# Sanoojan/VFace

Measured on AMD Instinct MI355X. Metric: swapped frames/sec at 512x512, 50-step DDIM, higher is better.
Workload: dtype f16

## Files before the change

### include/vface_hip.h

```cpp
#ifndef VFACE_HIP_H
#define VFACE_HIP_H

#include <stddef.h>
#include <stdint.h>

#ifdef __cplusplus
extern "C" {
#endif

#define VFACE_ABI_VERSION 7

#define VFACE_OK 0
#define VFACE_ERR_ARG (-1)
#define VFACE_ERR_ALIGN (-2)
#define VFACE_ERR_SHAPE (-3)
#define VFACE_ERR_DTYPE (-4)
#define VFACE_ERR_LAUNCH (-5)
#define VFACE_ERR_WORKSPACE (-6)

#define VFACE_F16 0
#define VFACE_BF16 1

#define VFACE_EPI_GEGLU 1
#define VFACE_EPI_OUT_F32 2
#define VFACE_TUNE_VARIANT(v) ((v) << 8)
#define VFACE_CONV_PAD_TRAILING 0x40000
#define VFACE_TUNE_NO_PERSISTENT 0x10000
#define VFACE_TUNE_PERSISTENT 0x20000
#define VFACE_TUNE_NO_PATCH 0x80000
#define VFACE_TUNE_PATCH 0x100000
#define VFACE_TUNE_GN8 0x8000000
#define VFACE_TUNE_NO_Q8 0x4000000
#define VFACE_TUNE_PATCH_BN160 0x2000000
#define VFACE_TUNE_F32_TRANSPOSE 0x1000000
#define VFACE_TUNE_BIG_TILE 0x10000000
#define VFACE_TUNE_NO_BIG_TILE 0x20000000
#define VFACE_TUNE_BIG_W256 0x200000
#define VFACE_TUNE_BIG_W320 0x400000

#define VFACE_FUSION_NONE 0
#define VFACE_FUSION_REPLACE 1
#define VFACE_FUSION_LINEAR 2

int vface_abi_version(void);
const char* vface_error_string(int code);
int vface_gemm_variants_built(void);

typedef struct vface_stream32 {
    const float* residual32;
    int64_t ldr32;
    float* out32;
    int64_t ldo32;
    const float* in_scale_shift;
    int64_t ld_scale_shift;
    int in_silu;
} vface_stream32;

int vface_gemm(const void* A, int64_t lda, const void* A2, int64_t lda2, int K1, int a2_row_mod, const void* Wt,
               int64_t ldw, int M, int N, int K, const float* bias, const float* rowbias, int rows_per_sample,
               int ld_rowbias, const void* residual, int64_t ldr, void* C, int64_t ldc, const void* zeros, int flags,
               int dtype, float* colstats, int64_t ld_colstats, void* workspace, int64_t workspace_bytes, void* stream,
               const vface_stream32* s32);

int64_t vface_splitk_workspace_bytes(int M, int N, int K, int flags, int rows_per_sample);

int vface_conv3x3(const void* X, int64_t ldx, int nimg, int H, int W, int Cin, const void* Wt, int64_t ldw, int Cout,
                  int stride, int upsample, const float* bias, const float* rowbias, int ld_rowbias,
                  const void* residual, int64_t ldr, void* Y, int64_t ldy, const void* zeros, int flags, int dtype,
                  float* colstats, int64_t ld_colstats, void* workspace, int64_t workspace_bytes, void* stream,
                  const vface_stream32* s32);

int vface_conv_uses_patch_kernel(int H, int W, int Cin, int Cout, int window, int stride, int upsample, int flags);

int vface_conv3x3_plus_1x1(const void* X, int64_t ldx, int nimg, int H, int W, int Cin, const void* X2, int64_t ldx2, int C2,
                           const void* Wt, int64_t ldw, int Cout, const float* bias, const float* rowbias, int ld_rowbias,
                           void* Y, int64_t ldy, const void* zeros, int flags, int dtype, float* colstats,
                           int64_t ld_colstats, void* workspace, int64_t workspace_bytes, void* stream,
                           const vface_stream32* s32);

int vface_upsample2x_conv3x3_phase(const void* X, int64_t ldx, int nimg, int H, int W, int Cin, const void* Wt, int64_t ldw,
                                   int Cout, int py, int px, const float* bias, const float* rowbias, int ld_rowbias, void* Y,
                                   int64_t ldy, const void* zeros, int flags, int dtype, float* colstats,
                                   int64_t ld_colstats, void* stream, const vface_stream32* s32);

int vface_attention(const void* Q, const void* K, const void* V, int64_t ldq, int64_t ldk, int64_t ldv, int64_t bsq,
                    int64_t bsk, int64_t bsv, const int32_t* qk_map, const int32_t* v_map, void* O, int64_t ldo,
                    int64_t bso, int B, int heads, int n, int nk, int dh, float scale, int dtype, int v_sets,
                    int set_stride, void* stream);
int vface_attention_shared_scores_supported(int dh, int v_sets);

int vface_layernorm(const void* x, int64_t ldx, const float* gamma, const float* beta, void* y, int64_t ldy, int M,
// ... 131 lines not shown
```

### vface_amd/csrc/gemm.hip

```cpp
#include <type_traits>

#include "common.hpp"
#include "vface_kernels.hpp"

namespace {

constexpr int BM = 128, BK = 64;
enum { MODE_PLAIN = 0, MODE_CONV_FAST = 1, MODE_CONV_GENERIC = 2 };

template <class TT, int MODE, int NT, bool DB, bool PERSIST, int RM = -1>
__global__ __launch_bounds__(256, 2) void gemm_kernel(GemmParams p) {
    using E = typename TT::elem;
    using V8 = typename TT::v8;
    constexpr int BN = 32 * NT;
    constexpr int BROUNDS = BN / 32;
    constexpr int A_ELEMS = BM * BK, B_ELEMS = BN * BK, STAGE = A_ELEMS + B_ELEMS;
    extern __shared__ __attribute__((aligned(16))) unsigned char smem_raw[];
    E* smem = reinterpret_cast<E*>(smem_raw);

    const int t = threadIdx.x;
    const int lane = t & 63;
    const int wave = __builtin_amdgcn_readfirstlane(t >> 6);
    const int wm = wave >> 1, wn = wave & 1;
    unsigned long long dbg_t0 = 0, dbg_t1 = 0, dbg_t2 = 0, dbg_e0 = 0, dbg_ew = 0, dbg_er = 0, dbg_es = 0;
// ... 800 lines not shown

template <class TT>
int launch_gemm(const GemmParams& p, int variant, hipStream_t stream) {
    if (p.mode == 0) return launch_mode<TT, MODE_PLAIN>(p, variant, stream);
    if (p.Cin % 64 == 0) return launch_mode<TT, MODE_CONV_FAST>(p, variant, stream);
    return launch_mode<TT, MODE_CONV_GENERIC>(p, variant, stream);
}

int pick_variant(const GemmParams& p) {
    const int forced = (p.flags >> 8) & 0xF;
    if (forced) return forced;
    const bool geglu = p.flags & GEMM_GEGLU;
    const long mref = p.rows_per_sample > 1 ? 24L * p.rows_per_sample : p.M;
    const long tiles160 = ((mref + BM - 1) / BM) * (p.N / 160);
    const bool n160 = !geglu && (p.N % 160 == 0) && ((p.N % 128 != 0) || tiles160 >= 1536);
    return n160 ? 6 : 5;
}

int split_for(int M, int N, int K, int flags, int rows_per_sample) {
    if (flags & (GEMM_GEGLU | GEMM_OUT_F32)) return 1;
    if ((N & 7) || ((flags >> 8) & 0xF) == 0xF) return 1;
    const bool n160 = (N % 160 == 0) && (N % 128 != 0);
    const int bn = n160 ? 160 : 128;
    const long mref = rows_per_sample > 1 ? 24L * rows_per_sample : M;
    const int tiles = (int)((mref + BM - 1) / BM) * ((N + bn - 1) / bn);
    const int nt = (K + BK - 1) / BK;
    if (tiles > 192 || nt < 16) return 1;
    int s = 512 / tiles;
    if (s > 8) s = 8;
    if (s > nt / 8) s = nt / 8;
    return s < 2 ? 1 : s;
}

}

int vf_launch_gemm_bf16(const GemmParams& p, int variant, hipStream_t stream);
#if defined(VF_GEMM_TU) && VF_GEMM_TU == 1
int vf_launch_gemm_bf16(const GemmParams& p, int variant, hipStream_t stream) { return launch_gemm<BF16>(p, variant, stream); }
#else
bool vf_gemm_variants_built() { return false; }

long vf_splitk_workspace_bytes(int M, int N, int K, int flags, int rows_per_sample) {
    int s = split_for(M, N, K, flags, rows_per_sample);
    if (s < 2) s = 0;
    if (rows_per_sample == 64 && (N % 128) == 0 && !(flags & (GEMM_GEGLU | GEMM_OUT_F32))) {
        int s8 = (int)(256 / (12L * (N / 128)));
        if (s8 > 8) s8 = 8;
        if (s8 < 1) s8 = 1;
        if (s8 > s) s = s8;
    }
    return (long)s * M * N * 4;
}

int vf_launch_gemm(const GemmParams& p_in, int dtype, hipStream_t stream) {
    GemmParams p = p_in;
    p.split_k = 1; p.kt_per_split = 0;
    if (!p.A || !p.Wt || (!p.C && !p.C32) || !p.zeros) return VF_ERR_ARG;
    if (p.M <= 0 || p.N <= 0 || p.K <= 0) return VF_ERR_ARG;
    if (p.res_f32 && !p.residual) p.res_f32 = 0;
    if (p.res_f32 || p.C32) {
        if ((p.flags & (GEMM_GEGLU | GEMM_OUT_F32 | GEMM_NARROW_EPILOGUE | 0x4000)) || (p.N & 7)) return VF_ERR_SHAPE;
        if (p.C32 && (((uintptr_t)p.C32 & 15) || (p.ldc32 & 3))) return VF_ERR_ALIGN;
        if (p.res_f32 && (((uintptr_t)p.residual & 15) || (p.ldr & 3))) return VF_ERR_ALIGN;
        if (p.out_phase && p.res_f32) return VF_ERR_SHAPE;
    }
    if ((p.K & 7) || (p.Kw & 7) || (p.lda & 7) || (p.ldw & 7) || (p.N & 3) || (p.ldc & 3)) return VF_ERR_ALIGN;
    if (((uintptr_t)p.A | (uintptr_t)p.Wt | (uintptr_t)p.zeros) & 15) return VF_ERR_ALIGN;
    if ((uintptr_t)p.C & 7) return VF_ERR_ALIGN;
    if (p.C32 && (((uintptr_t)p.C & 15) || (p.ldc & 7))) return VF_ERR_ALIGN;
    if (p.residual && (((uintptr_t)p.residual & 7) || (p.ldr & 3))) return VF_ERR_ALIGN;
    if (p.rowbias && (p.rows_per_sample <= 0 || (p.ld_rowbias & 3))) return VF_ERR_ARG;
    if ((p.flags & GEMM_GEGLU) && ((p.N & 31) || (p.flags & GEMM_OUT_F32) || p.residual || p.rowbias)) return VF_ERR_SHAPE;
    if (p.colstats && ((p.flags & (GEMM_GEGLU | GEMM_OUT_F32)) || (p.ld_colstats & 1) || ((uintptr_t)p.colstats & 15))) return VF_ERR_ARG;
    if (p.A2 && (p.K1 <= 0 || (p.K1 % BK) || (p.lda2 & 7) || ((uintptr_t)p.A2 & 15))) return VF_ERR_ALIGN;
    if (p.A2 && p.mode == 1 && ((p.Cin % 64) || ((p.K - p.K1) % BK) || p.upsample || p.a2_row_mod)) return VF_ERR_SHAPE;
    if (p.mode == 1) {
        if (p.ntaps == 0) { p.KH = p.KW = 3; p.ntaps = 9; p.pad_x = p.pad; }
        if (p.Cin <= 0 || (p.Cin & 7) || p.ntaps != p.KH * p.KW || p.ntaps > 9) return VF_ERR_SHAPE;
        if (p.A2 ? (p.K1 != p.ntaps * p.Cin || p.K <= p.K1) : (p.K != p.ntaps * p.Cin)) return VF_ERR_SHAPE;
        if (p.out_phase && (p.residual || (p.flags & GEMM_OUT_F32) || (p.N & 7))) return VF_ERR_SHAPE;
        if (p.out_phase && p.colstats && ((p.OH * p.OW) & 63)) return VF_ERR_SHAPE;
        if (p.stride != 1 && p.stride != 2) return VF_ERR_SHAPE;
    }
    {
        const unsigned long es = 2, lim = 0xFFFFFFF0ul;
        const unsigned long rows = p.mode == 1 ? (unsigned long)(p.M / (p.OH * p.OW)) * p.H * p.W : (unsigned long)p.M;
        const unsigned long ab = ((rows - 1) * (unsigned long)p.lda + (p.mode == 1 ? p.Cin : (p.A2 ? p.K1 : p.K))) * es;
        const unsigned long wb = ((unsigned long)(p.N - 1) * p.ldw + p.Kw) * es;
        unsigned long a2b = 0;
        if (p.A2) a2b = ((unsigned long)((p.a2_row_mod > 0 ? p.a2_row_mod : p.M) - 1) * p.lda2 + (p.K - p.K1)) * es;
        if (ab >= lim || wb >= lim || a2b >= lim) return VF_ERR_SHAPE;
        p.a_bytes = (unsigned)ab; p.w_bytes = (unsigned)wb; p.a2_bytes = (unsigned)a2b;
    }
    if (p.gn_ab) {
        if (p.mode != 1 || p.M <= 0) return VF_ERR_SHAPE;
        const unsigned long nimg = (unsigned long)(p.M / (p.OH * p.OW));
        const unsigned long gb = ((nimg - 1) * (unsigned long)p.ld_gn_ab + p.Cin) * 8ul;
        if (gb >= 0xFFFFFFF0ul) return VF_ERR_SHAPE;
        p.gn_ab_bytes = (unsigned)gb;
    }
    if (vf_conv_in16_ok(p)) return vf_launch_conv_in16(p, dtype, stream);
    int karg = 0;
    const int kchoice = vf_conv_kernel_choice(p, &karg);
    if (kchoice == 1) return vf_launch_conv_patch(p, dtype, stream);
    if (kchoice == 2 && p.workspace) {
        const int s = karg;
        if (s && p.workspace_bytes >= (long)s * p.M * p.N * 4 && !((uintptr_t)p.workspace & 15) && (p.M % 64) == 0 &&
            !(p.residual && (((uintptr_t)p.residual & 15) || (p.ldr & 7))) && !(p.ldc & 7) && !((uintptr_t)p.C & 15)) {
            p.split_k = s;
            const int rc = vf_launch_conv_q8(p, dtype, stream);
            if (rc != VF_OK) return rc;
            if (dtype == VF_DTYPE_F16) hipLaunchKernelGGL(splitk_reduce_kernel<F16>, dim3((p.M + 63) / 64, (p.N + 255) / 256), dim3(256), 0, stream, p);
            else hipLaunchKernelGGL(splitk_reduce_kernel<BF16>, dim3((p.M + 63) / 64, (p.N + 255) / 256), dim3(256), 0, stream, p);
            return hipGetLastError() == hipSuccess ? VF_OK : VF_ERR_LAUNCH;
        }
    }
    if (p.mode == 0 && (p.flags & GEMM_PATCH) && !((p.flags >> 8) & 0xF) && vf_gemm_patch_tile(p)) return vf_launch_gemm_patch(p, dtype, stream);
    if (p.mode == 0 && vf_gemm_big_choice(p)) return vf_launch_gemm_big(p, dtype, stream);
    if (p.gn_ab) return VF_ERR_SHAPE;
    const int variant = pick_variant(p);
    if ((p.res_f32 || p.C32) && variant != 5 && variant != 6) return VF_ERR_SHAPE;
    if (p.mode == 1 && (p.ntaps != 9 || p.out_phase || p.A2) && variant != 5 && variant != 6) return VF_ERR_SHAPE;
    if (p.workspace && !p.out_phase && (variant == 5 || variant == 6) && !((p.flags >> 8) & 0xF) && !(p.flags & 0x4000)) {
        const int s = split_for(p.M, p.N, p.K, p.flags, p.rows_per_sample);
        if (s > 1 && p.workspace_bytes >= (long)s * p.M * p.N * 4 && !((uintptr_t)p.workspace & 15) &&
            !(p.residual && (((uintptr_t)p.residual & 15) || (p.ldr & 7))) && !(p.ldc & 7) && !((uintptr_t)p.C & 15)) {
            const int nt = (p.K + BK - 1) / BK;
            p.split_k = s;
            p.kt_per_split = (nt + s - 1) / s;
            if ((long)(s - 1) * p.kt_per_split >= nt) p.split_k = (nt + p.kt_per_split - 1) / p.kt_per_split;
        }
    }
    if ((p.flags & GEMM_GEGLU) && (variant == 2 || variant == 4 || variant == 6 || variant == 8 || variant == 10)) return VF_ERR_SHAPE;
    if (p.colstats && (variant < 5 || variant > 8)) return VF_ERR_SHAPE;
    if ((variant >= 1 && variant <= 4) || variant == 9 || variant == 10) return VF_ERR_SHAPE;
    if (dtype == VF_DTYPE_F16) return launch_gemm<F16>(p, variant, stream);
    if (dtype == VF_DTYPE_BF16) return vf_launch_gemm_bf16(p, variant, stream);
    return VF_ERR_DTYPE;
}
#endif
```

### vface_amd/csrc/gemm_big.hip

```cpp
#include <type_traits>

#include "common.hpp"
#include "vface_kernels.hpp"

namespace {

constexpr int BM2 = 256, BN2 = 320;
constexpr int A_BYTES = BM2 * 128, B_BYTES = BN2 * 128, STAGE_BYTES = A_BYTES + B_BYTES;

template <class TT, int EPI, int NJ = 10>
__global__ __launch_bounds__(512, 2) void gemm256_kernel(GemmParams p) {
    static_assert(NJ == 10 || (NJ == 8 && EPI != 3), "channel tiles per wave");
    constexpr int BN2 = 32 * NJ, WN = 16 * NJ;
    constexpr int B_BYTES = BN2 * 128, STAGE_BYTES = A_BYTES + B_BYTES;
    constexpr int NPC = 4 + NJ / 2, NS = 2 * NJ;
    using E = typename TT::elem;
    using V8 = typename TT::v8;
    using V4 = typename TT::v4;
    extern __shared__ __attribute__((aligned(16))) unsigned char smem_raw[];
    const int t = threadIdx.x;
    const int lane = t & 63;
    const int wave = __builtin_amdgcn_readfirstlane(t >> 6);
    const int wm = wave >> 1, wn = wave & 1;
    const int fr = lane & 15, fq = lane >> 4;
    constexpr unsigned OOB = 0xFFFFFFF0u;

    const int ntn = p.N / BN2, ntm = (p.M + BM2 - 1) / BM2;
    int m0, n0;
    {
        const int nwg = ntn * ntm, id = blockIdx.x;
        const int q = nwg >> 3, r = nwg & 7, xcd = id & 7, loc = id >> 3;
        const int L = (xcd < r ? xcd * (q + 1) : r * (q + 1) + (xcd - r) * q) + loc;
        const int GN = p.tile_group > 0 ? p.tile_group : 8;
        const int g = L / (GN * ntm);
        const int rem = L - g * (GN * ntm);
        const int gw = min(GN, ntn - g * GN);
        const int tm = rem / gw;
        m0 = tm * BM2;
        n0 = (g * GN + (rem - tm * gw)) * BN2;
    }

    const float* rowbias_row = nullptr;
    if constexpr (EPI == 3) {
        const int rps = max(p.rows_per_sample, 1);
        const int smp = __builtin_amdgcn_readfirstlane(m0 / rps);
        rowbias_row = p.rowbias ? p.rowbias + (long)smp * p.ld_rowbias : nullptr;
    }
    const i32x4_t rA = raw_buffer_rsrc(p.A, p.a_bytes);
    const i32x4_t rA2 = raw_buffer_rsrc(p.A2 ? p.A2 : p.A, p.A2 ? p.a2_bytes : 0u);
    const i32x4_t rW = raw_buffer_rsrc(p.Wt, p.w_bytes);

    unsigned a_off[4], a2_off[4], b_off[NJ / 2];
#pragma unroll
    for (int i = 0; i < 4; ++i) {
        const int row = (wave + 8 * i) * 8 + (lane >> 3);
        const unsigned ch = (unsigned)((lane & 7) ^ ((row >> 1) & 7));
        const long m = m0 + row;
        a_off[i] = m < p.M ? (unsigned)((m * p.lda + ch * 8) * 2) : OOB;
        a2_off[i] = (p.A2 && m < p.M) ? (unsigned)((m * p.lda2 + ch * 8) * 2) : OOB;
    }
#pragma unroll
    for (int i = 0; i < NJ / 2; ++i) {
        const int row = (wave + 8 * i) * 8 + (lane >> 3);
        const unsigned ch = (unsigned)((lane & 7) ^ ((row >> 1) & 7));
        b_off[i] = (unsigned)((((long)(n0 + row)) * p.ldw + ch * 8) * 2);
    }
    const unsigned lds0 = lds_addr_of(smem_raw);
    auto issue_piece = [&](int s, int kt, int buf) {
        const unsigned kbase = (unsigned)kt * 64u;
        if (s < 4) {
            const bool second = p.A2 && (int)kbase >= p.K1;
            const unsigned base = second ? a2_off[s] : a_off[s];
            const unsigned off = base != OOB ? base + (second ? kbase - (unsigned)p.K1 : kbase) * 2u : OOB;
            const unsigned dst = lds0 + (unsigned)buf * STAGE_BYTES + (unsigned)(wave + 8 * s) * 1024u;
            if (second) raw_lds_dma16(rA2, dst, (int)off, 0);
            else raw_lds_dma16(rA, dst, (int)off, 0);
        } else {
            const unsigned dst = lds0 + (unsigned)buf * STAGE_BYTES + A_BYTES + (unsigned)(wave + 8 * (s - 4)) * 1024u;
            raw_lds_dma16(rW, dst, (int)(b_off[s - 4] + kbase * 2u), 0);
        }
    };

    f4_t acc[NJ][4];
#pragma unroll
    for (int j = 0; j < NJ; ++j)
#pragma unroll
        for (int i = 0; i < 4; ++i) acc[j][i] = f4_t{0.f, 0.f, 0.f, 0.f};

    const int arow = wm * 64 + fr, wrow = wn * WN + fr;
    const unsigned aadr = (unsigned)(arow * 128 + ((fq ^ ((arow >> 1) & 7)) << 4));
    const unsigned wadr = (unsigned)(A_BYTES + wrow * 128 + ((fq ^ ((wrow >> 1) & 7)) << 4));

    const int nt = p.K >> 6;
#pragma unroll
    for (int s = 0; s < NPC; ++s) issue_piece(s, 0, 0);
    if (nt > 1) { issue_piece(0, 1, 1); issue_piece(1, 1, 1); }
// ... 24 lines not shown
                if (s2 < NS) {
                    const int kk2 = s2 / NJ, j2 = s2 - kk2 * NJ;
                    wf[s2 & 3] = *reinterpret_cast<const V8*>(st + ((wadr + j2 * 2048) ^ (kk2 ? 64u : 0u)));
                } else if (more) {
                    wf[s2 & 3] = *reinterpret_cast<const V8*>(sn + wadr + (s2 - NS) * 2048);
                }
            }
            if (s == 4) {
#pragma unroll
                for (int i = 0; i < 4; ++i) af[1][i] = *reinterpret_cast<const V8*>(st + ((aadr + i * 2048) ^ 64u));
            }
            if (s == NS - 2 && more) {
#pragma unroll
                for (int i = 0; i < 4; ++i) af[0][i] = *reinterpret_cast<const V8*>(sn + aadr + i * 2048);
            }
            if (s >= NS - 2) { if (more2) issue_piece(s - (NS - 2), kt + 2, cur); }
            else if (s < NPC - 2) { if (more) issue_piece(s + 2, kt + 1, cur ^ 1); }
            __builtin_amdgcn_sched_barrier(0);
            __builtin_amdgcn_s_setprio(1);
#pragma unroll
            for (int i = 0; i < 4; ++i) acc[j][i] = TT::mfma32(wf[s & 3], af[kk][i], acc[j][i]);
            __builtin_amdgcn_s_setprio(0);
            __builtin_amdgcn_sched_barrier(0);
        }
    }

    __syncthreads();
    {
    int te = threadIdx.x;
    asm volatile("" : "+v"(te));
    const int lane = te & 63, fr = lane & 15, fq = lane >> 4;
    const int wrow0 = m0 + wm * 64;
    {
        auto add_vec = [&](const float* vec) {
            const __amdgpu_buffer_rsrc_t rV = __builtin_amdgcn_make_buffer_rsrc(const_cast<void*>(vec ? (const void*)vec : p.Wt), 0, vec ? p.N * 4 : 0, 0x00020000);
#pragma unroll
            for (int jh = 0; jh < 2; ++jh) {
                constexpr int HJ = NJ / 2;
                f4_t bj[HJ];
#pragma unroll
                for (int j = 0; j < HJ; ++j)
                    bj[j] = __builtin_bit_cast(f4_t, __builtin_amdgcn_raw_buffer_load_b128(rV, (n0 + wn * WN + (jh * HJ + j) * 16 + fq * 4) * 4, 0, 0));
#pragma unroll
                for (int j = 0; j < HJ; ++j)
#pragma unroll
                    for (int i = 0; i < 4; ++i) {
                        acc[jh * HJ + j][i] += bj[j];
                        asm volatile("" : "+v"(acc[jh * HJ + j][i]));
                    }
                __builtin_amdgcn_sched_barrier(0);
            }
        };
        add_vec(p.bias);
        if constexpr (EPI == 3) {
            add_vec(rowbias_row);
        }
    }
    __builtin_amdgcn_sched_barrier(0);
    E* Cout = reinterpret_cast<E*>(p.C);
    if constexpr (EPI == 0 || EPI == 1) {
        constexpr int OW = EPI == 1 ? WN / 2 : WN;
        constexpr int CH = OW / 8;
        constexpr int SPH = OW * 2 + 16;
        constexpr int NIT = (16 * CH + 63) / 64;
        unsigned char* scr = smem_raw + wave * (16 * SPH);
        const int ncol0 = EPI == 1 ? ((n0 + wn * WN) >> 1) : (n0 + wn * WN);
        int rr[NIT], cc[NIT];
#pragma unroll
        for (int it = 0; it < NIT; ++it) {
            const int idx = lane + 64 * it;
            rr[it] = idx < 16 * CH ? idx / CH : -1;
            cc[it] = idx - (idx / CH) * CH;
        }
#pragma unroll
        for (int i = 0; i < 4; ++i) {
            unsigned char* hrow = scr + fr * SPH + fq * 8;
            if constexpr (EPI == 0) {
#pragma unroll
                for (int j = 0; j < NJ; ++j)
                    *reinterpret_cast<V4*>(hrow + j * 32) = V4{from_f32<E>(acc[j][i][0]), from_f32<E>(acc[j][i][1]), from_f32<E>(acc[j][i][2]), from_f32<E>(acc[j][i][3])};
            } else {
#pragma unroll
                for (int jj = 0; jj < NJ / 2; ++jj) {
                    const float a0 = acc[2 * jj][i][0], a1 = acc[2 * jj][i][1], a2 = acc[2 * jj][i][2], a3 = acc[2 * jj][i][3];
                    const float g0 = acc[2 * jj + 1][i][0], g1 = acc[2 * jj + 1][i][1], g2 = acc[2 * jj + 1][i][2], g3 = acc[2 * jj + 1][i][3];
                    *reinterpret_cast<V4*>(hrow + jj * 32) = V4{from_f32<E>(a0 * gelu_erf_f(g0)), from_f32<E>(a1 * gelu_erf_f(g1)),
                                                                from_f32<E>(a2 * gelu_erf_f(g2)), from_f32<E>(a3 * gelu_erf_f(g3))};
                }
            }
            V8 o[NIT];
#pragma unroll
            for (int it = 0; it < NIT; ++it) o[it] = *reinterpret_cast<const V8*>(scr + max(rr[it], 0) * SPH + cc[it] * 16);
#pragma unroll
            for (int it = 0; it < NIT; ++it) {
                const long m = wrow0 + i * 16 + rr[it];
                if (rr[it] >= 0 && m < p.M) *reinterpret_cast<V8*>(Cout + m * p.ldc + ncol0 + cc[it] * 8) = o[it];
            }
        }
    } else if constexpr (EPI == 3) {
        constexpr int SP = 84;
        float* scr = reinterpret_cast<float*>(smem_raw) + wave * (16 * SP);
        const __amdgpu_buffer_rsrc_t rR = __builtin_amdgcn_make_buffer_rsrc(const_cast<void*>(p.residual ? p.residual : p.Wt), 0, (int)(p.residual ? p.res_bytes : 0u), 0x00020000);
        const __amdgpu_buffer_rsrc_t rC = __builtin_amdgcn_make_buffer_rsrc(p.C ? p.C : const_cast<void*>(p.Wt), 0, (int)(p.C ? p.c_bytes : 0u), 0x00020000);
        const __amdgpu_buffer_rsrc_t rC32 = __builtin_amdgcn_make_buffer_rsrc(p.C32, 0, (int)p.c32_bytes, 0x00020000);
        const int rrow = lane / 10, rch = lane - rrow * 10;
        const bool act = lane < 60;
        const bool has_res = p.residual != nullptr, has_c16 = p.C != nullptr;
// ... 104 lines not shown
                r32[it][1] = __builtin_bit_cast(f4_t, __builtin_amdgcn_raw_buffer_load_b128(rR, (int)off, 16, 0));
            }
        };
#pragma unroll
        for (int i = 0; i < 4; ++i) {
            float* srow = scr + fr * SP + fq * 4;
#pragma unroll
            for (int j = 0; j < NJ; ++j)
                *reinterpret_cast<float4*>(srow + j * 16) = make_float4(acc[j][i][0], acc[j][i][1], acc[j][i][2], acc[j][i][3]);
            __builtin_amdgcn_sched_barrier(0);
            if (i == 0) {
#pragma unroll
                for (int it = 0; it < NPASS; ++it) load_res(0, it);
            }
#pragma unroll
            for (int it = 0; it < NPASS; ++it) {
                const unsigned char* lrd = reinterpret_cast<const unsigned char*>(scr) + lofs[it];
                const f4_t x0 = *reinterpret_cast<const f4_t*>(lrd), x1 = *reinterpret_cast<const f4_t*>(lrd + 16);
                const f4_t a = r32[it][0], b = r32[it][1];
                const long m = wrow0 + i * 16 + rr[it];
                V8 o;
                o[0] = from_f32<E>(x0[0] + a[0]); o[1] = from_f32<E>(x0[1] + a[1]); o[2] = from_f32<E>(x0[2] + a[2]); o[3] = from_f32<E>(x0[3] + a[3]);
                o[4] = from_f32<E>(x1[0] + b[0]); o[5] = from_f32<E>(x1[1] + b[1]); o[6] = from_f32<E>(x1[2] + b[2]); o[7] = from_f32<E>(x1[3] + b[3]);
                if (i + 1 < 4) load_res(i + 1, it);
                const unsigned off = m < p.M ? (unsigned)((m * p.ldc + ncol0 + cc[it] * 8) * 2) : OOB;
                __builtin_amdgcn_raw_buffer_store_b128(__builtin_bit_cast(i32x4_t, o), rC, (int)off, 0, 0);
                __builtin_amdgcn_sched_barrier(0);
            }
        }
    }
    }
}

template <class TT, int EPI, int NJ>
int launch_big(const GemmParams& p, hipStream_t stream) {
    auto kern = gemm256_kernel<TT, EPI, NJ>;
    static VfOncePerDevice attr_set;
    constexpr int BN = 32 * NJ;
    constexpr int lds = 2 * (A_BYTES + BN * 128);
    if (!attr_set.set_lds(reinterpret_cast<const void*>(kern), lds)) return VF_ERR_LAUNCH;
    const int ntn = p.N / BN, ntm = (p.M + BM2 - 1) / BM2;
    GemmParams q = p;
    {
        const double a_mt = (double)BM2 * p.K * 2.0, w_nt = (double)BN * p.K * 2.0;
        int gn = (int)(__builtin_sqrt((double)ntm * ntn / 8.0 * a_mt / w_nt) + 0.5);
        const int cap = (int)(2097152.0 / w_nt);
        if (gn > cap) gn = cap;
        q.tile_group = gn < 1 ? 1 : (gn > ntn ? ntn : gn);
    }
    hipLaunchKernelGGL(kern, dim3(ntn * ntm), dim3(512), lds, stream, q);
    return hipGetLastError() == hipSuccess ? VF_OK : VF_ERR_LAUNCH;
}

template <class TT, int EPI>
int launch_big_width(const GemmParams& p, hipStream_t stream) {
    if constexpr (EPI != 3) {
        bool w256 = false;
        if (p.N % 256 == 0 && !(p.flags & GEMM_BIG_W320)) {
            const long ntm = (p.M + BM2 - 1) / BM2;
            const long r320 = (ntm * (p.N / 320) + 255) / 256, r256 = (ntm * (p.N / 256) + 255) / 256;
            w256 = (p.flags & GEMM_BIG_W256) || (p.K <= 1280 && (double)r256 * 0.85 < (double)r320);
        }
        if (w256) return launch_big<TT, EPI, 8>(p, stream);
    }
    return launch_big<TT, EPI, 10>(p, stream);
}

template <class TT>
int launch_big_dtype(const GemmParams& p, hipStream_t stream) {
    if (p.C32) return launch_big_width<TT, 3>(p, stream);
    if (p.flags & GEMM_GEGLU) return launch_big_width<TT, 1>(p, stream);
    if (p.residual) return launch_big_width<TT, 2>(p, stream);
    return launch_big_width<TT, 0>(p, stream);
}

}

bool vf_gemm_big_ok(const GemmParams& p) {
    if (p.mode != 0 || p.out_phase || p.gn_ab || p.split_k > 1 || p.a2_row_mod) return false;
    if ((p.N % BN2) || (p.K & 63) || p.K < 128 || (p.Kw < p.K)) return false;
    if (p.A2 && ((p.K1 & 63) || p.K1 <= 0 || p.K1 >= p.K)) return false;
    if (p.flags & (GEMM_OUT_F32 | GEMM_NARROW_EPILOGUE | GEMM_F32_TRANSPOSE | 0x4000 | (0xF << 8))) return false;
    if (p.C32) {
        if (p.flags & GEMM_GEGLU) return false;
        if (((uintptr_t)p.C32 & 15) || (p.ldc32 & 3)) return false;
        if (p.rowbias && (p.rows_per_sample <= 0 || (p.rows_per_sample % BM2) || (p.ld_rowbias & 3) || ((uintptr_t)p.rowbias & 15))) return false;
        if (p.colstats && ((p.M & 63) || (p.ld_colstats & 1) || ((uintptr_t)p.colstats & 7))) return false;
    } else if (p.colstats || p.rowbias || !p.C) {
        return false;
    }
    if (p.C && (((uintptr_t)p.C & 15) || (p.ldc & 7))) return false;
    if ((p.lda & 7) || (p.ldw & 7)) return false;
    if (p.residual && ((p.flags & GEMM_GEGLU) || ((uintptr_t)p.residual & 15) || (p.ldr & (p.res_f32 ? 3 : 7)))) return false;
    if (p.residual && !p.res_f32 && p.C32) return false;
    if (p.bias && ((uintptr_t)p.bias & 15)) return false;
    return true;
}

bool vf_gemm_big_choice(const GemmParams& p) {
    if ((p.flags & GEMM_NO_BIG) || !vf_gemm_big_ok(p)) return false;
    if (p.flags & GEMM_BIG) return true;
    if (p.C32) return false;
    return (long)((p.M + BM2 - 1) / BM2) * (p.N / BN2) >= 192;
}

int vf_launch_gemm_big(const GemmParams& p_in, int dtype, hipStream_t stream) {
    if (!vf_gemm_big_ok(p_in)) return VF_ERR_SHAPE;
    GemmParams p = p_in;
    {
        const unsigned long nout = (p.flags & GEMM_GEGLU) ? (unsigned long)p.N / 2 : (unsigned long)p.N;
        const unsigned long cb = p.C ? ((unsigned long)(p.M - 1) * p.ldc + nout) * 2ul : 0ul;
        const unsigned long rb = p.residual ? ((unsigned long)(p.M - 1) * p.ldr + p.N) * (p.res_f32 ? 4ul : 2ul) : 0ul;
        const unsigned long c32b = p.C32 ? ((unsigned long)(p.M - 1) * p.ldc32 + p.N) * 4ul : 0ul;
        if (cb >= 0xFFFFFFF0ul || rb >= 0xFFFFFFF0ul || c32b >= 0xFFFFFFF0ul) return VF_ERR_SHAPE;
        p.c_bytes = (unsigned)cb; p.res_bytes = (unsigned)rb; p.c32_bytes = (unsigned)c32b;
    }
    if (dtype == VF_DTYPE_F16) return launch_big_dtype<F16>(p, stream);
    if (dtype == VF_DTYPE_BF16) return launch_big_dtype<BF16>(p, stream);
    return VF_ERR_DTYPE;
}
```

### vface_amd/csrc/vface_kernels.hpp

```cpp
#pragma once
#include <hip/hip_runtime.h>
#include <stdint.h>

#include <atomic>

struct VfOncePerDevice {
    std::atomic<unsigned long long> done{0};
    bool set_lds(const void* kern, int bytes) {
        int dev = 0;
        if (hipGetDevice(&dev) != hipSuccess) return false;
        const unsigned long long bit = 1ull << (dev & 63);
        if (done.load(std::memory_order_acquire) & bit) return true;
        if (hipFuncSetAttribute(kern, hipFuncAttributeMaxDynamicSharedMemorySize, bytes) != hipSuccess) return false;
        done.fetch_or(bit, std::memory_order_release);
        return true;
    }
};

enum { GEMM_GEGLU = 1, GEMM_OUT_F32 = 2, GEMM_NO_XCD_REMAP = 0x1000, GEMM_NO_SETPRIO = 0x2000, GEMM_NARROW_EPILOGUE = 0x8000, GEMM_NO_PERSIST = 0x10000, GEMM_PERSIST = 0x20000,
       GEMM_NO_PATCH = 0x80000, GEMM_PATCH = 0x100000, GEMM_GN8 = 0x8000000 , GEMM_NO_Q8 = 0x4000000 , GEMM_PATCH_BN160 = 0x2000000 , GEMM_F32_TRANSPOSE = 0x1000000 ,
       GEMM_BIG = 0x10000000 , GEMM_NO_BIG = 0x20000000 ,
       GEMM_BIG_W256 = 0x200000 , GEMM_BIG_W320 = 0x400000  };

struct GemmParams {
    int mode;
    const void* A;
    long lda;
    const void* A2;
    long lda2;
    int K1, a2_row_mod;
    const void* Wt;
    long ldw;
    int Kw;
    int M, N, K;
    int H, W, Cin, OH, OW, stride, upsample;
    int pad;
    int pad_x;
    int KH, KW, ntaps;
    int out_phase;
    const float* bias;
    const float* rowbias;
    int rows_per_sample;
    int ld_rowbias;
    const void* residual;
    long ldr;
    void* C;
    long ldc;
    int res_f32;
    float* C32;
    long ldc32;
    const float* gn_ab;
    long ld_gn_ab;
    int gn_silu;
    unsigned gn_ab_bytes;
    const void* zeros;
    int flags;
    unsigned a_bytes, a2_bytes, w_bytes;
    float* colstats;
    long ld_colstats;
    float* workspace;
    long workspace_bytes;
    int split_k, kt_per_split;
    int tile_group;
    unsigned res_bytes, c_bytes, c32_bytes;
};
long vf_splitk_workspace_bytes(int M, int N, int K, int flags, int rows_per_sample);
bool vf_gemm_variants_built();
int vf_launch_gemm(const GemmParams& p, int dtype, hipStream_t stream);
int vf_conv_patch_tile(const GemmParams& p);
int vf_conv_kernel_choice(const GemmParams& p, int* arg);
int vf_launch_conv_patch(const GemmParams& p, int dtype, hipStream_t stream);
int vf_gemm_patch_tile(const GemmParams& p);
int vf_launch_gemm_patch(const GemmParams& p, int dtype, hipStream_t stream);
bool vf_gemm_big_ok(const GemmParams& p);
bool vf_gemm_big_choice(const GemmParams& p);
int vf_launch_gemm_big(const GemmParams& p, int dtype, hipStream_t stream);
bool vf_conv_in16_ok(const GemmParams& p);
int vf_launch_conv_in16(const GemmParams& p, int dtype, hipStream_t stream);
int vf_conv_q8_split(const GemmParams& p);
int vf_launch_conv_q8(const GemmParams& p, int dtype, hipStream_t stream);
bool vf_attention_shared_scores_supported(int dh, int v_sets);

struct FfnParams {
    const float* x32; long ldx;
    const float* gamma; const float* beta; float eps;
    const void* W1;
    const float* b1;
    const void* W2p;
    const float* b2;
    void* out16; long ldo;
    float* out32; long ldo32;
    int M, C;
    const void* att; long ldatt;
    const float* resid; long ldr;
    const float* bo;
    const float* rowbias; long ld_rowbias; int rows_per_sample;
    int Wpo_in_stream;
    const float* b_po;
    const float* x_in; long ld_xin;
    float* colstats; long ld_colstats;
};
bool vf_ffn_fused_supported(long M, int C);
int vf_launch_ffn_fused(const FfnParams& p, int dtype, hipStream_t stream);

struct LinearSmallParams {
    const void* a; long lda;
    const void* W; long ldw;
    const float* bias;
    void* out; long ldo; int out_f32;
    int silu;
    int M, N, K;
};
bool vf_linear_small_supported(int M, int N, int K);
int vf_launch_linear_small(const LinearSmallParams& p, int dtype, hipStream_t stream);

struct StFrontParams {
    const float* x32; long ldx;
    const float* ab; long ld_ab;
    int hw;
    const void* Wcat;
    const float* b_in;
    const float* gamma; const float* beta; float eps;
    float* t0; long ldt0;
    void* qkv; long ldq;
    void* ln; long ldln;
    int M, C, NQ;
    int rows_full, nq_lo;
    int gridA;
// ... 101 lines not shown
```

### vface_amd/hip.py

```python
from __future__ import annotations

import ctypes as C
import os
from typing import Optional

import torch

_HERE = os.path.dirname(os.path.abspath(__file__))
LIB_PATH = os.environ.get("VFACE_HIP_LIB") or os.path.join(_HERE, "lib", "libvface_hip.so")

F16, BF16 = 0, 1
EPI_GEGLU, EPI_OUT_F32 = 1, 2
CONV_PAD_TRAILING = 0x40000
TUNE_NO_PATCH, TUNE_PATCH = 0x80000, 0x100000
TUNE_GN8 = 0x8000000
TUNE_NO_Q8 = 0x4000000
TUNE_PATCH_BN160 = 0x2000000
TUNE_F32_TRANSPOSE = 0x1000000
TUNE_NO_PERSISTENT, TUNE_PERSISTENT = 0x10000, 0x20000
TUNE_BIG_W256, TUNE_BIG_W320 = 0x200000, 0x400000
TUNE_BIG_TILE, TUNE_NO_BIG_TILE = 0x10000000, 0x20000000
FUSION_NONE, FUSION_REPLACE, FUSION_LINEAR = 0, 1, 2

_i64, _i32, _f32, _vp, _sz = C.c_int64, C.c_int, C.c_float, C.c_void_p, C.c_size_t


class Stream32(C.Structure):
    _fields_ = [("residual32", _vp), ("ldr32", _i64), ("out32", _vp), ("ldo32", _i64),
                ("in_scale_shift", _vp), ("ld_scale_shift", _i64), ("in_silu", _i32)]


_s32p = C.POINTER(Stream32)

SIGNATURES = {
    "vface_abi_version": (C.c_int, []),
    "vface_error_string": (C.c_char_p, [_i32]),
    "vface_gemm_variants_built": (C.c_int, []),
    "vface_gemm": (C.c_int, [_vp, _i64, _vp, _i64, _i32, _i32, _vp, _i64, _i32, _i32, _i32, _vp, _vp, _i32, _i32, _vp,
                             _i64, _vp, _i64, _vp, _i32, _i32, _vp, _i64, _vp, _i64, _vp, _s32p]),
    "vface_conv3x3": (C.c_int, [_vp, _i64, _i32, _i32, _i32, _i32, _vp, _i64, _i32, _i32, _i32, _vp, _vp, _i32, _vp,
                                _i64, _vp, _i64, _vp, _i32, _i32, _vp, _i64, _vp, _i64, _vp, _s32p]),
    "vface_splitk_workspace_bytes": (_i64, [_i32, _i32, _i32, _i32, _i32]),
    "vface_conv_uses_patch_kernel": (C.c_int, [_i32, _i32, _i32, _i32, _i32, _i32, _i32, _i32]),
    "vface_conv3x3_plus_1x1": (C.c_int, [_vp, _i64, _i32, _i32, _i32, _i32, _vp, _i64, _i32, _vp, _i64, _i32, _vp, _vp, _i32,
                                         _vp, _i64, _vp, _i32, _i32, _vp, _i64, _vp, _i64, _vp, _s32p]),
    "vface_upsample2x_conv3x3_phase": (C.c_int, [_vp, _i64, _i32, _i32, _i32, _i32, _vp, _i64, _i32, _i32, _i32, _vp, _vp, _i32,
                                                 _vp, _i64, _vp, _i32, _i32, _vp, _i64, _vp, _s32p]),
    "vface_groupnorm_finalize_cols": (C.c_int, [_vp, _i64, _i32, _i32, _i32, _i32, _f32, _vp, _vp]),
    "vface_attention": (C.c_int, [_vp, _vp, _vp, _i64, _i64, _i64, _i64, _i64, _i64, _vp, _vp, _vp, _i64, _i64, _i32,
                                  _i32, _i32, _i32, _i32, _f32, _i32, _i32, _i32, _vp]),
    "vface_attention_shared_scores_supported": (C.c_int, [_i32, _i32]),
    "vface_layernorm": (C.c_int, [_vp, _i64, _vp, _vp, _vp, _i64, _i32, _i32, _f32, _i32, _i32, _vp]),
    "vface_groupnorm_partial_floats": (C.c_int, [_i32, _i32, _i32, _i32]),
    "vface_groupnorm_stats": (C.c_int, [_vp, _i64, _i32, _i32, _i32, _i32, _f32, _vp, _vp, _i32, _i32, _vp]),
    "vface_groupnorm_coeffs_from_cols": (C.c_int, [_vp, _i64, _i32, _i32, _i32, _i32, _f32, _vp, _vp, _vp, _vp]),
    "vface_groupnorm_apply": (C.c_int, [_vp, _i64, _vp, _vp, _vp, _vp, _i64, _i32, _i32, _i32, _i32, _i32, _i32, _i32, _vp]),
    "vface_flow_warp": (C.c_int, [_vp, _i64, _i64, _vp, _i64, _vp, _vp, _vp, _i64, _i64, _i32, _i32, _i32, _i32, _f32,
                                  _f32, _i32, _vp, _vp, _i32, _vp]),
    "vface_flow_to_latent": (C.c_int, [_vp, _vp, _i32, _i32, _i32, _i32, _vp]),
    "vface_im2col": (C.c_int, [_vp, _i64, _i32, _i32, _i32, _i32, _i32, _i32, _i32, _i32, _i32, _vp, _i64, _i32, _vp]),
    "vface_channel_stats_partial_floats": (_i64, [_i32, _i32, _i32]),
    "vface_channel_stats": (C.c_int, [_vp, _i64, _i32, _i32, _i32, _f32, _vp, _vp, _i32, _vp]),
    "vface_channel_norm_act": (C.c_int, [_vp, _i64, _vp, _vp, _i64, _vp, _i64, _vp, _i64, _i64, _i32, _i32, _i32, _i32, _vp]),
    "vface_gru_gate": (C.c_int, [_vp, _i64, _vp, _vp, _i64, _vp, _i64, _i64, _i32, _i32, _vp]),
    "vface_gru_update": (C.c_int, [_vp, _i64, _vp, _i64, _vp, _vp, _i64, _vp, _i64, _i64, _i32, _i32, _vp]),
    "vface_avgpool2_f32": (C.c_int, [_vp, _vp, _i64, _i32, _i32, _vp]),
    "vface_corr_lookup": (C.c_int, [_vp, _vp, _vp, _i32, _vp, _i32, _i32, _f32, _vp, _i64, _i64, _i32, _vp]),
    "vface_flow_update": (C.c_int, [_vp, _vp, _i64, _vp, _i64, _vp, _i64, _vp, _i64, _i64, _i32, _vp]),
    "vface_convex_upsample": (C.c_int, [_vp, _i64, _vp, _vp, _i32, _i32, _i32, _f32, _vp]),
    "vface_frame_to_u8": (C.c_int, [_vp, _vp, _i32, _i32, _i32, _i32, _vp]),
    "vface_resample_u8": (C.c_int, [_vp, _vp, _i32, _i32, _i32, _i32, _i32, _vp, _vp, _i32, _vp]),
    "vface_perspective_paste": (C.c_int, [_vp, _i32, _i32, _vp, _i32, _i32, _i32, _vp, _vp, _vp]),
    "vface_frame_normalise_resize": (C.c_int, [_vp, _i32, _i32, _vp, _i32, _i32, _i32, _vp]),
    "vface_attn1_workspace_bytes": (_sz, [_i32, _i32, _i32, _i32]),
# ... 599 lines not shown
```

Baseline: 8.597.

## Split big-tile GEMM rows to run wave-quantization tail on 128-row kernel

Adds a cost-model planner that splits a large GEMM along M. Full rounds of 256x320 (or 256x256) tiles go to the big kernel, and the leftover partial round goes to the 128-row kernel with a suitable variant. The aim is to cut wave-quantization waste in the last partial round of big tiles. It also extends the big kernel with a residual+rowbias epilogue (EPI 4) so more GEMMs qualify. In exchange it adds an extra launch and relies on hardcoded timing constants that may not match real shapes.

```diff
diff --git a/include/vface_hip.h b/include/vface_hip.h
--- a/include/vface_hip.h
+++ b/include/vface_hip.h
@@ -37,6 +37,8 @@
 #define VFACE_TUNE_NO_BIG_TILE 0x20000000
 #define VFACE_TUNE_BIG_W256 0x200000
 #define VFACE_TUNE_BIG_W320 0x400000
+#define VFACE_TUNE_ROW_SPLIT 0x40
+#define VFACE_TUNE_NO_ROW_SPLIT 0x80
 
 #define VFACE_FUSION_NONE 0
 #define VFACE_FUSION_REPLACE 1
diff --git a/vface_amd/csrc/gemm.hip b/vface_amd/csrc/gemm.hip
--- a/vface_amd/csrc/gemm.hip
+++ b/vface_amd/csrc/gemm.hip
@@ -876,6 +876,29 @@
     return (long)s * M * N * 4;
 }
 
+static int launch_rows128(GemmParams p, int dtype, hipStream_t stream) {
+    if (p.gn_ab) return VF_ERR_SHAPE;
+    const int variant = pick_variant(p);
+    if ((p.res_f32 || p.C32) && variant != 5 && variant != 6) return VF_ERR_SHAPE;
+    if (p.mode == 1 && (p.ntaps != 9 || p.out_phase || p.A2) && variant != 5 && variant != 6) return VF_ERR_SHAPE;
+    if (p.workspace && !p.out_phase && (variant == 5 || variant == 6) && !((p.flags >> 8) & 0xF) && !(p.flags & 0x4000)) {
+        const int s = split_for(p.M, p.N, p.K, p.flags, p.rows_per_sample);
+        if (s > 1 && p.workspace_bytes >= (long)s * p.M * p.N * 4 && !((uintptr_t)p.workspace & 15) &&
+            !(p.residual && (((uintptr_t)p.residual & 15) || (p.ldr & 7))) && !(p.ldc & 7) && !((uintptr_t)p.C & 15)) {
+            const int nt = (p.K + BK - 1) / BK;
+            p.split_k = s;
+            p.kt_per_split = (nt + s - 1) / s;
+            if ((long)(s - 1) * p.kt_per_split >= nt) p.split_k = (nt + p.kt_per_split - 1) / p.kt_per_split;
+        }
+    }
+    if ((p.flags & GEMM_GEGLU) && (variant == 2 || variant == 4 || variant == 6 || variant == 8 || variant == 10)) return VF_ERR_SHAPE;
+    if (p.colstats && (variant < 5 || variant > 8)) return VF_ERR_SHAPE;
+    if ((variant >= 1 && variant <= 4) || variant == 9 || variant == 10) return VF_ERR_SHAPE;
+    if (dtype == VF_DTYPE_F16) return launch_gemm<F16>(p, variant, stream);
+    if (dtype == VF_DTYPE_BF16) return vf_launch_gemm_bf16(p, variant, stream);
+    return VF_ERR_DTYPE;
+}
+
 int vf_launch_gemm(const GemmParams& p_in, int dtype, hipStream_t stream) {
     GemmParams p = p_in;
     p.split_k = 1; p.kt_per_split = 0;
@@ -940,26 +963,32 @@
         }
     }
     if (p.mode == 0 && (p.flags & GEMM_PATCH) && !((p.flags >> 8) & 0xF) && vf_gemm_patch_tile(p)) return vf_launch_gemm_patch(p, dtype, stream);
-    if (p.mode == 0 && vf_gemm_big_choice(p)) return vf_launch_gemm_big(p, dtype, stream);
-    if (p.gn_ab) return VF_ERR_SHAPE;
-    const int variant = pick_variant(p);
-    if ((p.res_f32 || p.C32) && variant != 5 && variant != 6) return VF_ERR_SHAPE;
-    if (p.mode == 1 && (p.ntaps != 9 || p.out_phase || p.A2) && variant != 5 && variant != 6) return VF_ERR_SHAPE;
-    if (p.workspace && !p.out_phase && (variant == 5 || variant == 6) && !((p.flags >> 8) & 0xF) && !(p.flags & 0x4000)) {
-        const int s = split_for(p.M, p.N, p.K, p.flags, p.rows_per_sample);
-        if (s > 1 && p.workspace_bytes >= (long)s * p.M * p.N * 4 && !((uintptr_t)p.workspace & 15) &&
-            !(p.residual && (((uintptr_t)p.residual & 15) || (p.ldr & 7))) && !(p.ldc & 7) && !((uintptr_t)p.C & 15)) {
-            const int nt = (p.K + BK - 1) / BK;
-            p.split_k = s;
-            p.kt_per_split = (nt + s - 1) / s;
-            if ((long)(s - 1) * p.kt_per_split >= nt) p.split_k = (nt + p.kt_per_split - 1) / p.kt_per_split;
-        }
-    }
-    if ((p.flags & GEMM_GEGLU) && (variant == 2 || variant == 4 || variant == 6 || variant == 8 || variant == 10)) return VF_ERR_SHAPE;
-    if (p.colstats && (variant < 5 || variant > 8)) return VF_ERR_SHAPE;
-    if ((variant >= 1 && variant <= 4) || variant == 9 || variant == 10) return VF_ERR_SHAPE;
-    if (dtype == VF_DTYPE_F16) return launch_gemm<F16>(p, variant, stream);
-    if (dtype == VF_DTYPE_BF16) return vf_launch_gemm_bf16(p, variant, stream);
-    return VF_ERR_DTYPE;
+    if (p.mode == 0) {
+        int tail_variant = 0;
+        int lead = vf_gemm_round_plan(p, &tail_variant);
+        if (lead > 0 && lead < p.M && p.workspace && !p.out_phase && split_for(p.M, p.N, p.K, p.flags, p.rows_per_sample) > 1)
+            lead = vf_gemm_big_choice(p) ? p.M : 0;
+        if (lead >= p.M) return vf_launch_gemm_big(p, dtype, stream);
+        if (lead > 0) {
+            const unsigned long es = 2;
+            GemmParams a = p, b = p;
+            a.M = lead; b.M = p.M - lead;
+            b.A = static_cast<const char*>(p.A) + (unsigned long)lead * p.lda * es;
+            if (p.A2) b.A2 = static_cast<const char*>(p.A2) + (unsigned long)lead * p.lda2 * es;
+            b.C = static_cast<char*>(p.C) + (unsigned long)lead * p.ldc * es;
+            if (p.residual) b.residual = static_cast<const char*>(p.residual) + (unsigned long)lead * p.ldr * (p.res_f32 ? 4ul : 2ul);
+            if (p.rowbias) b.rowbias = p.rowbias + (long)(lead / p.rows_per_sample) * p.ld_rowbias;
+            for (GemmParams* q : {&a, &b}) {
+                q->a_bytes = (unsigned)(((unsigned long)(q->M - 1) * p.lda + (p.A2 ? p.K1 : p.K)) * es);
+                q->a2_bytes = p.A2 ? (unsigned)(((unsigned long)(q->M - 1) * p.lda2 + (p.K - p.K1)) * es) : 0u;
+            }
+            const int rc = vf_launch_gemm_big(a, dtype, stream);
+            if (rc != VF_OK) return rc;
+            b.workspace = nullptr; b.workspace_bytes = 0;
+            if (tail_variant) b.flags |= tail_variant << 8;
+            return launch_rows128(b, dtype, stream);
+        }
+    }
+    return launch_rows128(p, dtype, stream);
 }
 #endif
diff --git a/vface_amd/csrc/gemm_big.hip b/vface_amd/csrc/gemm_big.hip
--- a/vface_amd/csrc/gemm_big.hip
+++ b/vface_amd/csrc/gemm_big.hip
@@ -6,11 +6,13 @@
 namespace {
 
 constexpr int BM2 = 256, BN2 = 320;
+constexpr int BIG_SLOTS = 256;
 constexpr int A_BYTES = BM2 * 128, B_BYTES = BN2 * 128, STAGE_BYTES = A_BYTES + B_BYTES;
 
 template <class TT, int EPI, int NJ = 10>
 __global__ __launch_bounds__(512, 2) void gemm256_kernel(GemmParams p) {
     static_assert(NJ == 10 || (NJ == 8 && EPI != 3), "channel tiles per wave");
+    constexpr bool ROWBIAS = EPI == 3 || EPI == 4;
     constexpr int BN2 = 32 * NJ, WN = 16 * NJ;
     constexpr int B_BYTES = BN2 * 128, STAGE_BYTES = A_BYTES + B_BYTES;
     constexpr int NPC = 4 + NJ / 2, NS = 2 * NJ;
@@ -41,7 +43,7 @@
     }
 
     const float* rowbias_row = nullptr;
-    if constexpr (EPI == 3) {
+    if constexpr (ROWBIAS) {
         const int rps = max(p.rows_per_sample, 1);
         const int smp = __builtin_amdgcn_readfirstlane(m0 / rps);
         rowbias_row = p.rowbias ? p.rowbias + (long)smp * p.ld_rowbias : nullptr;
@@ -172,7 +174,7 @@
             }
         };
         add_vec(p.bias);
-        if constexpr (EPI == 3) {
+        if constexpr (ROWBIAS) {
             add_vec(rowbias_row);
         }
     }
@@ -383,16 +385,16 @@
     return hipGetLastError() == hipSuccess ? VF_OK : VF_ERR_LAUNCH;
 }
 
+bool big_width_256(const GemmParams& p, long ntm) {
+    if (p.C32 || (p.N % 256) || (p.flags & GEMM_BIG_W320)) return false;
+    const long r320 = (ntm * (p.N / 320) + BIG_SLOTS - 1) / BIG_SLOTS, r256 = (ntm * (p.N / 256) + BIG_SLOTS - 1) / BIG_SLOTS;
+    return (p.flags & GEMM_BIG_W256) || (p.K <= 1280 && (double)r256 * 0.85 < (double)r320);
+}
+
 template <class TT, int EPI>
 int launch_big_width(const GemmParams& p, hipStream_t stream) {
     if constexpr (EPI != 3) {
-        bool w256 = false;
-        if (p.N % 256 == 0 && !(p.flags & GEMM_BIG_W320)) {
-            const long ntm = (p.M + BM2 - 1) / BM2;
-            const long r320 = (ntm * (p.N / 320) + 255) / 256, r256 = (ntm * (p.N / 256) + 255) / 256;
-            w256 = (p.flags & GEMM_BIG_W256) || (p.K <= 1280 && (double)r256 * 0.85 < (double)r320);
-        }
-        if (w256) return launch_big<TT, EPI, 8>(p, stream);
+        if (big_width_256(p, (p.M + BM2 - 1) / BM2)) return launch_big<TT, EPI, 8>(p, stream);
     }
     return launch_big<TT, EPI, 10>(p, stream);
 }
@@ -401,7 +403,7 @@
 int launch_big_dtype(const GemmParams& p, hipStream_t stream) {
     if (p.C32) return launch_big_width<TT, 3>(p, stream);
     if (p.flags & GEMM_GEGLU) return launch_big_width<TT, 1>(p, stream);
-    if (p.residual) return launch_big_width<TT, 2>(p, stream);
+    if (p.residual) return p.rowbias ? launch_big_width<TT, 4>(p, stream) : launch_big_width<TT, 2>(p, stream);
     return launch_big_width<TT, 0>(p, stream);
 }
 
@@ -417,8 +419,10 @@
         if (((uintptr_t)p.C32 & 15) || (p.ldc32 & 3)) return false;
         if (p.rowbias && (p.rows_per_sample <= 0 || (p.rows_per_sample % BM2) || (p.ld_rowbias & 3) || ((uintptr_t)p.rowbias & 15))) return false;
         if (p.colstats && ((p.M & 63) || (p.ld_colstats & 1) || ((uintptr_t)p.colstats & 7))) return false;
-    } else if (p.colstats || p.rowbias || !p.C) {
+    } else if (p.colstats || !p.C) {
         return false;
+    } else if (p.rowbias) {
+        if (!p.residual || p.rows_per_sample <= 0 || (p.rows_per_sample % BM2) || (p.ld_rowbias & 3) || ((uintptr_t)p.rowbias & 15)) return false;
     }
     if (p.C && (((uintptr_t)p.C & 15) || (p.ldc & 7))) return false;
     if ((p.lda & 7) || (p.ldw & 7)) return false;
@@ -433,6 +437,40 @@
     if (p.flags & GEMM_BIG) return true;
     if (p.C32) return false;
     return (long)((p.M + BM2 - 1) / BM2) * (p.N / BN2) >= 192;
+}
+
+constexpr double BIG_T0_320 = 18.5, BIG_T1_320 = 2.17, BIG_T0_256 = 16.6, BIG_T1_256 = 1.69;
+constexpr double ROW128_T0_160 = 14.8, ROW128_T1_160 = 1.20, ROW128_T0_128 = 10.2, ROW128_T1_128 = 1.16;
+constexpr double EXTRA_LAUNCH_US = 5.0;
+int vf_gemm_round_plan(const GemmParams& p, int* tail_variant) {
+    if (tail_variant) *tail_variant = 0;
+    const bool big = vf_gemm_big_choice(p);
+    const int whole = big ? p.M : 0;
+    if ((p.flags & (GEMM_NO_BIG | GEMM_NO_ROW_SPLIT)) || !vf_gemm_big_ok(p)) return whole;
+    if (p.split_k > 1 || p.C32 || p.colstats || p.a2_row_mod) return whole;
+    const long ntm = (p.M + BM2 - 1) / BM2;
+    const long spt = p.rowbias ? p.rows_per_sample / BM2 : 1;
+    long lead = 0;
+    if (p.flags & GEMM_ROW_SPLIT) {
+        lead = ntm / 2 / spt * spt;
+    } else {
+        if (!big) return 0;
+        const bool w256 = big_width_256(p, ntm);
+        const long ntn = p.N / (w256 ? 256 : 320);
+        const long rounds = (ntm * ntn + BIG_SLOTS - 1) / BIG_SLOTS;
+        lead = (rounds - 1) * BIG_SLOTS / ntn / spt * spt;
+        if (lead <= 0 || lead >= ntm) return whole;
+        const double kt = p.K / 64.0;
+        const double t_big = w256 ? BIG_T0_256 + BIG_T1_256 * kt : BIG_T0_320 + BIG_T1_320 * kt;
+        const double lead_rounds = (double)((lead * ntn + BIG_SLOTS - 1) / BIG_SLOTS);
+        const long mt128 = (p.M - lead * BM2 + 127) / 128;
+        const double r160 = (p.N % 160 == 0 && !(p.flags & GEMM_GEGLU)) ? (double)((mt128 * (p.N / 160) + 2 * BIG_SLOTS - 1) / (2 * BIG_SLOTS)) * (ROW128_T0_160 + ROW128_T1_160 * kt) : 1e30;
+        const double r128 = (double)((mt128 * ((p.N + 127) / 128) + 2 * BIG_SLOTS - 1) / (2 * BIG_SLOTS)) * (ROW128_T0_128 + ROW128_T1_128 * kt);
+        const double cut = lead_rounds * t_big + (r160 < r128 ? r160 : r128) + EXTRA_LAUNCH_US;
+        if (!(cut + EXTRA_LAUNCH_US < (double)rounds * t_big)) return whole;
+        if (tail_variant && r160 < r128) *tail_variant = 6;
+    }
+    return (lead <= 0 || lead >= ntm) ? whole : (int)(lead * BM2);
 }
 
 int vf_launch_gemm_big(const GemmParams& p_in, int dtype, hipStream_t stream) {
diff --git a/vface_amd/csrc/vface_kernels.hpp b/vface_amd/csrc/vface_kernels.hpp
--- a/vface_amd/csrc/vface_kernels.hpp
+++ b/vface_amd/csrc/vface_kernels.hpp
@@ -20,7 +20,8 @@
 enum { GEMM_GEGLU = 1, GEMM_OUT_F32 = 2, GEMM_NO_XCD_REMAP = 0x1000, GEMM_NO_SETPRIO = 0x2000, GEMM_NARROW_EPILOGUE = 0x8000, GEMM_NO_PERSIST = 0x10000, GEMM_PERSIST = 0x20000,
        GEMM_NO_PATCH = 0x80000, GEMM_PATCH = 0x100000, GEMM_GN8 = 0x8000000 , GEMM_NO_Q8 = 0x4000000 , GEMM_PATCH_BN160 = 0x2000000 , GEMM_F32_TRANSPOSE = 0x1000000 ,
        GEMM_BIG = 0x10000000 , GEMM_NO_BIG = 0x20000000 ,
-       GEMM_BIG_W256 = 0x200000 , GEMM_BIG_W320 = 0x400000  };
+       GEMM_BIG_W256 = 0x200000 , GEMM_BIG_W320 = 0x400000 ,
+       GEMM_ROW_SPLIT = 0x40 , GEMM_NO_ROW_SPLIT = 0x80  };
 
 struct GemmParams {
     int mode;
@@ -74,6 +75,7 @@
 int vf_launch_gemm_patch(const GemmParams& p, int dtype, hipStream_t stream);
 bool vf_gemm_big_ok(const GemmParams& p);
 bool vf_gemm_big_choice(const GemmParams& p);
+int vf_gemm_round_plan(const GemmParams& p, int* tail_variant);
 int vf_launch_gemm_big(const GemmParams& p, int dtype, hipStream_t stream);
 bool vf_conv_in16_ok(const GemmParams& p);
 int vf_launch_conv_in16(const GemmParams& p, int dtype, hipStream_t stream);
diff --git a/vface_amd/hip.py b/vface_amd/hip.py
--- a/vface_amd/hip.py
+++ b/vface_amd/hip.py
@@ -20,6 +20,7 @@
 TUNE_NO_PERSISTENT, TUNE_PERSISTENT = 0x10000, 0x20000
 TUNE_BIG_W256, TUNE_BIG_W320 = 0x200000, 0x400000
 TUNE_BIG_TILE, TUNE_NO_BIG_TILE = 0x10000000, 0x20000000
+TUNE_ROW_SPLIT, TUNE_NO_ROW_SPLIT = 0x40, 0x80
 FUSION_NONE, FUSION_REPLACE, FUSION_LINEAR = 0, 1, 2
 
 _i64, _i32, _f32, _vp, _sz = C.c_int64, C.c_int, C.c_float, C.c_void_p, C.c_size_t
```

New measurement: 8.619 (median of 6 runs). About the same (+0.2%).
